# tachitachi/SR-WaveNet

Measured on NVIDIA B200. Metric: audio samples/sec, higher is better.
Workload: dtype f16

## Files before the change

sr-wavenet_b200/csrc/fused.cu:

```cuda
#include "common.cuh"
#include "mol.cuh"
#include "umma.cuh"
#include "philox.cuh"
#include <cuda_fp16.h>
#include <algorithm>
#include <cstdlib>

namespace fused {

constexpr int kTile = 128;
__host__ __device__ constexpr int tiles_of(bool teacher) { return teacher ? 3 : 4; }
__host__ __device__ constexpr int chunk_of(bool teacher) { return kTile * tiles_of(teacher); }
constexpr int kHalo = 512;
constexpr int kMaxLayers = 40;
constexpr int kMaxSeg = 8;

constexpr int kWfBytes = 64 * 32 * 2;
constexpr int kWrsTeacher = 32 * 160 * 2;
constexpr int kWrsStudent = 32 * 32 * 2;
constexpr int kH1Bytes = 128 * 128 * 2;
constexpr int kH2Bytes = 128 * 32 * 2;

struct Seg { int b, t_start, t_out, t_end; };

// ... 18 lines not shown
  int* err;
#ifdef SRWN_TUNING
  long long* trace;
  int trace_chunk;
#endif
  int T, L, P, frames, O, M;
  int ring_bytes_per_team;
  int dil[kMaxLayers];
  int ring_off[kMaxLayers];
  int rsuf[kMaxLayers + 1];
};

template <bool TEACHER>
struct SmemMapT {
  static constexpr int NT = tiles_of(TEACHER);
  static constexpr int rows = kHalo + NT * kTile;
  static constexpr int hbuf = 0;
  static constexpr int hbuf_bytes = 4 * rows * 16;
  static constexpr int cbuf = hbuf + 2 * hbuf_bytes;
  static constexpr int cbuf_bytes = 4 * kTile * 16;
  static constexpr int wst = cbuf + NT * cbuf_bytes;
  static constexpr int wst_bytes = kWfBytes + (TEACHER ? kWrsTeacher : kWrsStudent);
  static constexpr int head = wst + 2 * wst_bytes;
  static constexpr int bias = head + (TEACHER ? kH1Bytes + kH2Bytes : 0);
  static constexpr int hbias = bias + kMaxLayers * 32 * 4;
  static constexpr int front = hbias + (128 + 128 + 32 + 64 + 4) * 4;
  static constexpr int cbs = front + 64 * 4;
  static constexpr int bars = cbs + NT * (kMaxLayers + 1) * 32 * 4;
  static constexpr int n_bars = 40;
  static constexpr int misc = bars + n_bars * 8;
  static constexpr int total = misc + 64;
};
static_assert(SmemMapT<true>::total <= 232448 && SmemMapT<false>::total <= 232448, "shared memory budget");
static_assert(3 * 16 * kTile * 16 <= 2 * SmemMapT<true>::hbuf_bytes, "head operand overlay");

template <int NT>
struct BarT {
  static constexpr int D1 = 0;
  static constexpr int D2 = NT;
  static constexpr int HD = 2 * NT;
  static constexpr int WFULL = 4 * NT;
  static constexpr int WEMPTY = WFULL + 2;
  static constexpr int HALO = WFULL + 4;
  static constexpr int G1 = WFULL + 6;
  static constexpr int HDD = WFULL + 8;
  static constexpr int TAIL = HDD + NT;
  static constexpr int C2 = TAIL + 1;
  static constexpr int count = C2 + 2 * NT;
};
static_assert(BarT<3>::count <= 40 && BarT<4>::count <= 40, "barrier slots");

using namespace umma;

__device__ __forceinline__ uint32_t gate2(f2_t a) {
  float a0, a1;
  upk(a, a0, a1);
  const f2_t f = pk(tanh_fast(a0), tanh_fast(a1));
  const f2_t s = mul2(f, f);
  f2_t t = fma2(s, pk(0.0017294071149080992f, 0.0017294071149080992f), pk(-0.020638039335608482f, -0.020638039335608482f));
  t = fma2(s, t, pk(0.2499687224626541f, 0.2499687224626541f));
  const f2_t c = fma2(f, pk(0.5f, 0.5f), mul2(s, t));
  float c0, c1;
  upk(c, c0, c1);
  return pack2(c0, c1);
}

__device__ __forceinline__ void store_row(uint8_t* buf, int rows_per_kc, int row, const float* v) {
#pragma unroll
  for (int kc = 0; kc < 4; kc++) {
    uint4 q;
    q.x = pack2(v[kc * 8 + 0], v[kc * 8 + 1]); q.y = pack2(v[kc * 8 + 2], v[kc * 8 + 3]);
    q.z = pack2(v[kc * 8 + 4], v[kc * 8 + 5]); q.w = pack2(v[kc * 8 + 6], v[kc * 8 + 7]);
    *reinterpret_cast<uint4*>(buf + ((size_t)kc * rows_per_kc + row) * 16) = q;
  }
}
__device__ __forceinline__ void store_row_packed(uint8_t* buf, int rows_per_kc, int row, const uint32_t* w) {
#pragma unroll
  for (int kc = 0; kc < 4; kc++)
    *reinterpret_cast<uint4*>(buf + ((size_t)kc * rows_per_kc + row) * 16) =
        make_uint4(w[kc * 4 + 0], w[kc * 4 + 1], w[kc * 4 + 2], w[kc * 4 + 3]);
}

#ifndef SRWN_TUNING
#define TRACE(role, layer, slot) do {} while (0)
#else
#define TRACE(role, layer, slot)                                                            \
  do {                                                                                      \
    if (tracing) p.trace[((role) * kMaxLayers + (layer)) * 12 + (slot)] = clock64();      \
  } while (0)
#endif

constexpr int kLoadWarp = 0;
__host__ __device__ constexpr int threads_of(bool handoff, int nt) { return (1 + 4 * nt + (handoff ? 1 : 0)) * 32; }

__device__ __noinline__ bool flag_spin(const uint32_t* f, uint32_t need, volatile int* abort_flag, const int* gerr, int code, long long limit) {
  const long long t0 = clock64();
  int spins = 0;
  uint32_t v;
  while (true) {
    __nanosleep(32);
    asm volatile("ld.acquire.gpu.global.u32 %0, [%1];" : "=r"(v) : "l"(f) : "memory");
    if (v >= need) return true;
    if (*abort_flag) return false;
    if (((++spins) & 1023) == 0 && *reinterpret_cast<const volatile int*>(gerr)) return false;
    if (clock64() - t0 > limit) {
      if (atomicCAS((int*)abort_flag, 0, 1) == 0) ((int*)abort_flag)[1] = code;
      return false;
    }
  }
}
__device__ __forceinline__ bool flag_try(const uint32_t* f, uint32_t need) {
  uint32_t v;
  asm volatile("ld.acquire.gpu.global.u32 %0, [%1];" : "=r"(v) : "l"(f) : "memory");
  if (v < need) return false;
  asm volatile("fence.proxy.async;" ::: "memory");
  return true;
}
__device__ __forceinline__ bool flag_wait(const uint32_t* f, uint32_t need, volatile int* abort_flag, const int* gerr, int code, long long limit) {
  uint32_t v;
  asm volatile("ld.acquire.gpu.global.u32 %0, [%1];" : "=r"(v) : "l"(f) : "memory");
  if (v < need && !flag_spin(f, need, abort_flag, gerr, code, limit)) return false;
// ... 84 lines not shown

  const int G = p.G, team = (int)blockIdx.x / G, member = (int)blockIdx.x % G;
  const Seg* segs = p.segs + (size_t)team * kMaxSeg;
  const int nseg = p.nseg[team];
  uint8_t* ring = p.rings + (size_t)team * p.ring_bytes_per_team;
  uint32_t* flags = p.flags + (size_t)team * kMaxLayers;
  const uint32_t ringcnt = sbase + SM::misc + 16;
  uint32_t pub_expect = 0;
  int seq = 0;
  int u0e = 0, u0o = 0, lay_base = 0;
  int chunk_idx = 0;
  int head_idx = 0;
  int tail_idx = 0;
  double nll_acc = 0.0;
  const bool elected = elect_one();

  for (int si = 0; si < nseg; si++) {
    const Seg sg = segs[si];
    for (int t0 = sg.t_start; t0 < sg.t_end; t0 += CH) {
      const int n = seq++;
      if (n % G != member) continue;
      const bool warm = TEACHER ? (t0 + CH <= sg.t_out) : false;
      const bool do_head = TEACHER && !warm;
      int Lc = L;
      if (t0 + CH <= sg.t_out) {
        const int dist = sg.t_out - (t0 + CH);
        Lc = 0;
        while (Lc < L && p.rsuf[Lc + 1] > dist) Lc++;
        if (Lc < 1) Lc = 1;
      }
#define U0(par) ((par) ? u0o : u0e)
#ifdef SRWN_TUNING
      const bool tracing_chunk = p.trace != nullptr && blockIdx.x == 0 && chunk_idx == p.trace_chunk;
#else
      constexpr bool tracing_chunk = false; (void)tracing_chunk;
#endif

      if (warp == kLoadWarp) {
        bool have_next = false;
        for (int l = 0; l < Lc; l++) {
          const int s = l & 1;
          const int use = U0(s) + (l >> 1);
          [[maybe_unused]] const bool tracing = tracing_chunk && lane == 0;
          TRACE(6, l, 0);
          if (l >= 2 && !mbar_wait(bar(BAR_G1 + s), (use - 1) & 1, abort_flag, 0x1100000 | l, p.wait_limit)) break;
          TRACE(6, l, 2);
          if (HANDOFF && n > 0 && !have_next &&
              !flag_wait(flags + l, (uint32_t)n, abort_flag, p.err, 0x1200000 | l, p.wait_limit)) break;
          have_next = false;
          const int d = p.dil[l];
          const uint8_t* rl = ring + p.ring_off[l];
          const uint32_t dst0 = sbase + SM::hbuf + s * SM::hbuf_bytes;
          const int slot0 = (int)((unsigned)t0 % (unsigned)d);
          if (t0 - d >= sg.t_start) {
            if (lane == 0) {
              mbar_expect_tx(bar(BAR_HALO + s), (uint32_t)(4 * d * 16));
              const uint32_t n1 = (uint32_t)(d - slot0) * 16, n2 = (uint32_t)slot0 * 16;
#pragma unroll
              for (int kc = 0; kc < 4; kc++) {
                const uint32_t dst = dst0 + (uint32_t)(kc * ROWS + kHalo - d) * 16;
                const uint8_t* src = rl + (size_t)kc * d * 16;
                asm volatile("cp.async.bulk.shared::cluster.global.mbarrier::complete_tx::bytes [%0], [%1], %2, [%3];"
                             ::"r"(dst), "l"(src + (size_t)slot0 * 16), "r"(n1), "r"(bar(BAR_HALO + s)) : "memory");
                if (n2)
                  asm volatile("cp.async.bulk.shared::cluster.global.mbarrier::complete_tx::bytes [%0], [%1], %2, [%3];"
                               ::"r"(dst + n1), "l"(src), "r"(n2), "r"(bar(BAR_HALO + s)) : "memory");
// ... 40 lines not shown
            const int rows = ring_rows_of(p.dil[r], lane, CH);
            if (rows) {
              pub_expect += (uint32_t)rows;
              if ((int32_t)(ld_acquire_cta_shared(ringcnt + 4 * lane) - pub_expect) < 0) {
                const long long t0 = clock64();
                while ((int32_t)(ld_acquire_cta_shared(ringcnt + 4 * lane) - pub_expect) < 0) {
                  __nanosleep(128);
                  if (*abort_flag) { ok = false; break; }
                  if (clock64() - t0 > p.wait_limit) {
                    if (atomicCAS((int*)abort_flag, 0, 1) == 0) ((int*)abort_flag)[1] = 0x4000000 | (lane << 8) | r;
                    ok = false; break;
                  }
                }
              }
            }
          }
          ok = __all_sync(0xffffffffu, ok);
          if (ok && lane == 0) flag_publish(flags + r, (uint32_t)n + 1);
        }
        if (ok && lane == 0)
          for (int r = last + 1; r < L; r++) flag_publish(flags + r, (uint32_t)n + 1);
      } else {
        const int gw = warp & 3, m = (((warp - 1) >> 2) + gw + 1) % NT;
        const bool issuer = gw == m;
        const bool leader = issuer && elected;
        const int row = gw * 32 + lane;
        const uint32_t lane_addr = (uint32_t)(gw * 32) << 16;
        const int t = t0 + m * kTile + row;
        const bool in_utt = t < p.T;
        int frame = (t0 + m * kTile) / p.P;
        if (frame > p.frames - 1) frame = p.frames - 1;
        const float* cb_g = p.cb + ((size_t)sg.b * p.frames + frame) * (size_t)(L + 1) * 32;
        float* cb = reinterpret_cast<float*>(smem + SM::cbs) + m * (kMaxLayers + 1) * 32;
        for (int i = row; i < (L + 1) * 32; i += kTile) cb[i] = __ldg(cb_g + i);
        group_sync(m);
        const float* s_bias = reinterpret_cast<const float*>(smem + SM::bias);
        const float* s_front = reinterpret_cast<const float*>(smem + SM::front);
        const int rc = m * kTile + row;
        f2_t h2[16];
        float v[32];
        uint32_t w16[16];
        bool alive = true;
        [[maybe_unused]] const bool tracing = tracing_chunk && row == 0;
        constexpr uint32_t id32 = make_idesc(0, 128, 32), id128 = make_idesc(0, 128, 128);
        const uint32_t hb_lo0 = ((sbase + SM::hbuf) >> 4) + (uint32_t)(kHalo + m * kTile) + ((uint32_t)ROWS << 16);
        const uint32_t wb_lo0 = (sbase + SM::wst) >> 4;
        const uint32_t d_conv = tmem + m * TCOLS, d_skip = tmem + m * TCOLS + 32;
        uint32_t d_cop = d_skip;
        constexpr bool kLateG1 = !TEACHER && !HANDOFF;
        constexpr bool kLateWempty = !TEACHER && HANDOFF;

        {
          auto x_at = [&](int tt) -> float {
            const size_t i = (size_t)sg.b * p.T + tt;
            if (!TEACHER && p.noise.on) return philox::logistic_at(p.noise.seed, p.noise.stream, (uint64_t)i);
            return __ldg(p.x_in + i);
          };
          const float xm1 = (t >= 1 && t - 1 < p.T) ? x_at(t - 1) : 0.f;
          const float xm2 = (t >= 2 && t - 2 < p.T) ? x_at(t - 2) : 0.f;
#pragma unroll
          for (int j = 0; j < 16; j++) {
            const float a = fmaf(xm2, s_front[2 * j], fmaf(xm1, s_front[32 + 2 * j], cb[2 * j]));
            const float b = fmaf(xm2, s_front[2 * j + 1], fmaf(xm1, s_front[32 + 2 * j + 1], cb[2 * j + 1]));
            h2[j] = pk(a, b);
            w16[j] = pack2(a, b);
          }
          alive = mbar_wait(bar(BAR_HALO + 0), U0(0) & 1, abort_flag, 0x2000000 | (m << 8), p.wait_limit);
          store_row_packed(smem + SM::hbuf, ROWS, kHalo + rc, w16);
          const int d0 = p.dil[0];
          fence_async_smem();
          mbar_arrive(bar(BAR_HD + 2 * m + 0));
          if (rc >= CH - d0) store_row_packed(ring + p.ring_off[0], d0, t % d0, w16);
        }

        for (int l = 0; l < Lc; l++) {
          const int s = l & 1, sn = s ^ 1;
          const uint32_t ph = (lay_base + l) & 1, phs = (U0(s) + (l >> 1)) & 1;
          TRACE(m, l, 0);
          const uint32_t hb_lo = hb_lo0 + (uint32_t)(s * (SM::hbuf_bytes >> 4));
          const uint32_t wb_lo = wb_lo0 + (uint32_t)(s * (SM::wst_bytes >> 4));
          const uint32_t dl = (uint32_t)p.dil[l];
          const uint32_t b1_lo = wb_lo + (32u << 16);
          const uint32_t b2_lo = wb_lo + (kWfBytes >> 4) + ((uint32_t)wrs_rows << 16);
          if (gw == ((m + 3) & 3)) {
            alive = mbar_wait(bar(BAR_WFULL + s), phs, abort_flag, 0x3000000 | (m << 8) | l, p.wait_limit) && alive;
            if (NT > 3 && m >= 3) alive = mbar_wait(bar(BAR_HD + 2 * (m - 3) + s), phs, abort_flag, 0x3300000 | (m << 8) | l, p.wait_limit) && alive;
          }
          if (gw == ((m + 1) & 3) && m >= 1) alive = mbar_wait(bar(BAR_HD + 2 * (m - 1) + s), phs, abort_flag, 0x3100000 | (m << 8) | l, p.wait_limit) && alive;
          if (gw == ((m + 2) & 3) && m >= 2) alive = mbar_wait(bar(BAR_HD + 2 * (m - 2) + s), phs, abort_flag, 0x3200000 | (m << 8) | l, p.wait_limit) && alive;
          group_sync(m);
          TRACE(m, l, 1);
          if (HANDOFF && gw == (m == 0 ? 1 : 0) && lane == 0) {
            const int rows = ring_rows_of((int)dl, m, CH);
            if (rows) ring_rows_done(ringcnt + 4 * m, (uint32_t)rows);
          }
          if (issuer) {
            tc_fence_after();
            if (leader) {
              tc_mma<0>(d_conv, desc_from_lo(hb_lo - dl), desc_from_lo(b1_lo), id32);
              tc_mma<1>(d_conv, desc_from_lo(hb_lo - dl + 2 * ROWS), desc_from_lo(b1_lo + 64), id32);
              tc_mma<1>(d_conv, desc_from_lo(hb_lo), desc_from_lo(b1_lo + 128), id32);
              tc_mma<1>(d_conv, desc_from_lo(hb_lo + 2 * ROWS), desc_from_lo(b1_lo + 192), id32);
              tc_commit(bar(BAR_D1 + m));
              if constexpr (!kLateG1) tc_commit(bar(BAR_G1 + s));
            }
            __syncwarp();
          }
          TRACE(m, l, 2);
          bool next_ok = true;
          if (l + 1 < Lc && !issuer) {
            if (l >= 1) next_ok = mbar_poll(bar(BAR_G1 + sn), (U0(sn) + ((l - 1) >> 1)) & 1);
// ... 65 lines not shown
          TRACE(m, l, 9);
          if (l + 1 < L) {
#pragma unroll
            for (int j = 0; j < 16; j++) { float a, b; upk(h2[j], a, b); w16[j] = pack2(a, b); }
            if (l + 1 < Lc) {
              if (!next_ok) {
                if (l >= 1) alive = mbar_wait(bar(BAR_G1 + sn), (U0(sn) + ((l - 1) >> 1)) & 1, abort_flag, 0x2300000 | (m << 8) | l, p.wait_limit) && alive;
                alive = mbar_wait(bar(BAR_HALO + sn), (U0(sn) + ((l + 1) >> 1)) & 1, abort_flag, 0x2400000 | (m << 8) | l, p.wait_limit) && alive;
              }
              TRACE(m, l, 10);
              store_row_packed(smem + SM::hbuf + sn * SM::hbuf_bytes, ROWS, kHalo + rc, w16);
              tc_fence_before();
              fence_async_smem();
              mbar_arrive(bar(BAR_HD + 2 * m + sn));
            } else {
              tc_fence_before();
              alive = mbar_wait(bar(BAR_TAIL), tail_idx & 1, abort_flag, 0x2700000 | (m << 8) | l, p.wait_limit) && alive;
            }
            const int dn = p.dil[l + 1];
            if (rc >= CH - dn) store_row_packed(ring + p.ring_off[l + 1], dn, t % dn, w16);
            TRACE(m, l, 11);
          } else {
            tc_fence_before();
          }
        }

        if (TEACHER) {
          if (do_head) {
            const float* s_hb = reinterpret_cast<const float*>(smem + SM::hbias);
            uint8_t* a3 = smem + SM::hbuf + m * (16 * kTile * 16);
            const uint32_t a3_lo = ((sbase + SM::hbuf + m * (16 * kTile * 16)) >> 4) + ((uint32_t)kTile << 16);
            alive = mbar_wait(bar(BAR_G1 + ((L - 1) & 1)), (U0((L - 1) & 1) + ((L - 1) >> 1)) & 1, abort_flag, 0x2500000 | (m << 8), p.wait_limit) && alive;
            alive = mbar_wait(bar(BAR_WEMPTY + ((L - 1) & 1)), (U0((L - 1) & 1) + ((L - 1) >> 1)) & 1, abort_flag, 0x2510000 | (m << 8), p.wait_limit) && alive;
            tc_fence_after();
#pragma unroll 1
            for (int hs = 0; hs < 2; hs++) {
              for (int q = 0; q < 4; q++) {
                tc_ld32(d_skip + lane_addr + q * 32, v);
                tc_wait_ld();
#pragma unroll
                for (int j = 0; j < 32; j++) v[j] = fmaxf(v[j] + s_hb[hs * 128 + q * 32 + j], 0.f);
                store_row(a3 + (size_t)q * 4 * kTile * 16, kTile, row, v);
              }
              tc_fence_before();
              fence_async_smem();
              group_sync(m);
              if (issuer) {
                tc_fence_after();
                if (leader && !*abort_flag) {
                  const uint32_t wlo = ((sbase + SM::head + (hs == 0 ? 0 : kH1Bytes)) >> 4) + ((uint32_t)(hs == 0 ? 128 : 32) << 16);
                  const int nrows = hs == 0 ? 128 : 32;
#pragma unroll
                  for (int j = 0; j < 8; j++)
                    tc_mma_dyn(hs == 0 ? d_skip : d_conv, desc_from_lo(a3_lo + 2 * j * kTile), desc_from_lo(wlo + 2 * j * nrows),
                               hs == 0 ? id128 : id32, j);
                  tc_commit(bar(BAR_HDD + m));
                }
                __syncwarp();
              }
              alive = mbar_wait(bar(BAR_HDD + m), (head_idx * 2 + hs) & 1, abort_flag, 0x2600000 | (m << 8) | hs, p.wait_limit) && alive;
              tc_fence_after();
            }
            tc_ld32(d_conv + lane_addr, v);
            tc_wait_ld();
            tc_fence_before();
            if (alive && in_utt && t >= sg.t_out) {
#pragma unroll
              for (int j = 0; j < 32; j++) v[j] += s_hb[256 + j];
              const size_t at = (size_t)sg.b * p.T + t;
              float nl = 0.f;
              if (p.x_scored) {
                const float xs = __ldg(p.x_scored + at);
                if (p.M == 5) nl = mol_nll_fixed<5>(xs, v);
                else {
                  float lg[32];
#pragma unroll
                  for (int j = 0; j < 32; j++) lg[j] = v[j];
                  nl = mol_nll_one(xs, lg, p.M);
                }
              }
              if (p.logits_out) {
                float* dst = p.logits_out + at * p.O;
                if (p.O == 20) {
#pragma unroll
                  for (int j = 0; j < 5; j++)
                    reinterpret_cast<float4*>(dst)[j] = make_float4(v[4 * j], v[4 * j + 1], v[4 * j + 2], v[4 * j + 3]);
                } else {
#pragma unroll
                  for (int j = 0; j < 32; j++) if (j < p.O) dst[j] = v[j];
                }
              }
              if (p.x_scored) {
                if (p.nll_out) p.nll_out[at] = nl;
                nll_acc += (double)nl;
              }
            }
          }
        } else {
          const float* s_hb = reinterpret_cast<const float*>(smem + SM::hbias);
          const float* hk = s_hb + 288;
          float p0 = 0.f, p1 = 0.f;
#pragma unroll
          for (int j = 0; j < 16; j++) {
            float a, b;
            upk(h2[j], a, b);
            const float e0 = fmaxf(a, 0.f), e1 = fmaxf(b, 0.f);
            p0 = fmaf(e0, hk[4 * j], p0); p1 = fmaf(e0, hk[4 * j + 1], p1);
            p0 = fmaf(e1, hk[4 * j + 2], p0); p1 = fmaf(e1, hk[4 * j + 3], p1);
          }
          if (alive && in_utt && t >= sg.t_out) {
            const size_t at = (size_t)sg.b * p.T + t;
            const float sc = expf(p0 + hk[64]);
            const float mu = p1 + hk[65];
            p.scale_out[at] = sc;
            p.mean_out[at] = mu;
            const float xin = p.noise.on ? philox::logistic_at(p.noise.seed, p.noise.stream, (uint64_t)at) : __ldg(p.x_in + at);
            p.x_out[at] = fmaf(xin, sc, mu);
          }
        }
      }
      if (HANDOFF && Lc < L && warp != kLoadWarp && warp != kPubWarp) {
        const int gw = warp & 3, m = (((warp - 1) >> 2) + gw + 1) % NT;
        group_sync(m);
        if (gw == (m == 0 ? 1 : 0) && lane == 0) {
          const int rows = ring_rows_of(p.dil[Lc], m, CH);
          if (rows) ring_rows_done(ringcnt + 4 * m, (uint32_t)rows);
        }
      }
      if (do_head) head_idx++;
      if (Lc < L) tail_idx++;
      chunk_idx++;
      u0e += (Lc + 1) >> 1; u0o += Lc >> 1; lay_base += Lc;
      tc_fence_before();
      asm volatile("fence.proxy.async;" ::: "memory");
      __syncthreads();
      tc_fence_after();
      if (*abort_flag) break;
    }
    if (*abort_flag) break;
  }

  if (TEACHER && p.nll_partial) {
    double* s_red = reinterpret_cast<double*>(smem + SM::cbuf);
    for (int s = 16; s >= 1; s >>= 1) nll_acc += __shfl_xor_sync(0xffffffffu, nll_acc, s);
    if (lane == 0) s_red[warp] = nll_acc;
    __syncthreads();
    if (tid == 0) {
      double tot = 0;
      for (int w = 1; w <= 4 * NT; w++) tot += s_red[w];
      p.nll_partial[blockIdx.x] = tot;
    }
  }
  if (tid == 0 && *abort_flag) {
    volatile int* e = p.err;
    e[1] = abort_flag[1]; e[2] = chunk_idx; e[3] = blockIdx.x;
    __threadfence_system();
    e[0] = 1;
  }
  tc_fence_before();
  __syncthreads();
  if (warp == kLoadWarp) {
    tc_fence_after();
    asm volatile("tcgen05.dealloc.cta_group::1.sync.aligned.b32 %0, %1;" ::"r"(tmem), "r"(512));
  }
}

__global__ void k_sum_partials(const double* __restrict__ part, int n, float* __restrict__ out) {
  double tot = 0;
  for (int i = threadIdx.x; i < n; i += 32) tot += part[i];
// ... 236 lines not shown
    if (force_G > 0 && G != std::min(force_G, std::min(kMaxTeam, grid))) continue;
    int teams = grid / G;
    if ((long long)teams > total) teams = (int)total;
    if (teams < 1) continue;
    Partition cand = partition_for(B, T, kChunk, warm_cost, teams);
    const double lag = kLagLayers / L;
    const double period = std::max(1.0, G * lag);
    const double time = (cand.cost / G + (G > 1 ? 0.5 : 0.0)) * period * (G > 1 ? handoff_cost : 1.0) + (G - 1) * lag;
    if (time < best_time) { best_time = time; best = cand; best.G = G; }
  }
  return best;
}

struct FusedWs {
  float* cb; uint8_t* rings; uint32_t* flags; double* partial;
#ifdef SRWN_TUNING
  long long* trace;
#endif
  float *scales, *means, *xa, *xb;
  size_t bytes;
};

static FusedWs carve_fused(const srwn_ctx* c, int B, int T, void* ws, size_t cap) {
  WsCarver w(ws, cap);
  FusedWs r{};
  const size_t frames = T / c->cfg.pool_stride, L = c->cfg.n_layers, n = (size_t)B * T;
  const int grid = c->sm_count > 0 ? c->sm_count : 148;
  const size_t nst = c->cfg.kind == SRWN_STUDENT ? (size_t)c->cfg.num_flows : 1;
  r.cb = w.take<float>((size_t)B * frames * (L + 1) * 32 * nst);
  r.rings = w.take<uint8_t>((size_t)grid * ((size_t)c->sum_dilation * 64 + 256));
  r.flags = w.take<uint32_t>((size_t)grid * kMaxLayers * nst);
  r.partial = w.take<double>(grid);
#ifdef SRWN_TUNING
  r.trace = w.take<long long>(7 * kMaxLayers * 12);
#endif
  if (c->cfg.kind == SRWN_STUDENT) {
    r.scales = w.take<float>(n * c->cfg.num_flows);
    r.means = w.take<float>(n * c->cfg.num_flows);
    r.xa = w.take<float>(n);
    r.xb = w.take<float>(n);
  }
  r.bytes = w.used;
  return r;
}

size_t fused_partition_bytes(const srwn_ctx* c) {
  const size_t grid = c->sm_count > 0 ? c->sm_count : 148;
  return grid * kMaxSeg * sizeof(Seg) + grid * sizeof(int);
}

size_t fused_workspace_bytes(const srwn_ctx* c, int op, int B, int T) {
  return carve_fused(c, B, T, nullptr, 0).bytes;
}

template <bool TEACHER>
static int launch_fused(srwn_ctx* c, const Params& p, int grid, cudaStream_t st) {
  const bool handoff = p.G > 1;
  auto kern = handoff ? k_fused<TEACHER, true> : k_fused<TEACHER, false>;
  SRWN_CUDA(cudaFuncSetAttribute(kern, cudaFuncAttributeMaxDynamicSharedMemorySize, SmemMapT<TEACHER>::total));
  Params pl = p;
  void* args[] = {&pl};
  SRWN_CUDA(cudaLaunchCooperativeKernel((const void*)kern, dim3(grid), dim3(threads_of(handoff, tiles_of(TEACHER))), args, SmemMapT<TEACHER>::total, st));
  SRWN_LAUNCH_CHECK();
  return SRWN_OK;
}

static int sticky_error(const srwn_ctx* c) {
// ... 90 lines not shown
  for (int f = 0; f < F; f++) {
    Params p;
    int rc = prepare(c, f, enc, B, T, w, &p, &grid, f == 0, st);
    if (rc) return rc;
    float* xout = (f == F - 1 && x_last) ? x_last : ((f & 1) ? w.xb : w.xa);
    p.x_in = xin; p.scale_out = w.scales + (size_t)f * n; p.mean_out = w.means + (size_t)f * n; p.x_out = xout;
    if (f == 0) p.noise = noise;
    ProfScope prof(c, st, "k_fused<student,fp16>", 1);
    rc = launch_fused<false>(c, p, grid, st);
    if (rc) return rc;
    xin = xout;
  }
  return run_flow_compose(z, noise, z_out, w.scales, w.means, F, out, s_tot, mu_tot, (int64_t)n, st);
}

int fused_check_error(void* ws, size_t ws_bytes, const srwn_ctx* c, int B, int T, cudaStream_t st) {
  (void)ws; (void)ws_bytes; (void)B; (void)T;
  SRWN_CUDA(cudaStreamSynchronize(st));
  volatile int* e = c->h_err;
  if (e && e[0]) {
    const int code = e[1], chunk = e[2], cta = e[3];
    e[0] = 0; e[1] = 0; e[2] = 0; e[3] = 0;
    return srwn_fail(SRWN_ERR_CUDA, "fused kernel aborted: pipeline wait timed out (code 0x%x, chunk %d, cta %d)", code, chunk, cta);
  }
  return SRWN_OK;
}

void fused_last_partition(const srwn_ctx* c, int* teams, int* G) { *teams = c->part_teams; *G = c->part_G; }

#ifdef SRWN_TUNING
extern "C" int srwn_debug_read_trace(srwn_handle_t h, int32_t B, int32_t T, void* ws, size_t ws_bytes,
                                     long long* out, int32_t count) {
  FusedWs w = carve_fused(h, B, T, ws, ws_bytes);
  if (count > 7 * kMaxLayers * 12) count = 7 * kMaxLayers * 12;
  SRWN_CUDA(cudaDeviceSynchronize());
  SRWN_CUDA(cudaMemcpy(out, w.trace, sizeof(long long) * count, cudaMemcpyDeviceToHost));
  return SRWN_OK;
}

namespace fused {
template <int N, int CNT>
__device__ __forceinline__ void bench_issue(uint32_t tmem_col, uint32_t a_lo, uint32_t b_lo, uint32_t mbar_addr) {
  constexpr uint32_t idesc = make_idesc(0, 128, N);
#pragma unroll
  for (int i = 0; i < CNT; i++) {
    if (i == 0) tc_mma<0>(tmem_col, desc_from_lo(a_lo), desc_from_lo(b_lo), idesc);
    else tc_mma<1>(tmem_col, desc_from_lo(a_lo + (i & 3) * 256), desc_from_lo(b_lo + (i & 3) * 64), idesc);
  }
  tc_commit(mbar_addr);
}

__global__ void __launch_bounds__(416, 1) k_mma_bench(long long* out) {
  extern __shared__ __align__(1024) uint8_t smem[];
  __shared__ uint32_t tmem_slot;
  __shared__ __align__(8) uint64_t mbar[16];
  __shared__ long long s_t[16][2];
  const uint32_t sbase = smem_u32(smem);
  const int warp = threadIdx.x >> 5;
  for (int i = threadIdx.x; i < 65536 / 4; i += 416) reinterpret_cast<uint32_t*>(smem)[i] = 0x3c003c00u;
  if (threadIdx.x == 0) {
    for (int i = 0; i < 16; i++) mbar_init(smem_u32(&mbar[i]), 1);
    asm volatile("fence.mbarrier_init.release.cluster;" ::: "memory");
  }
  fence_async_smem();
  if (warp == 0) {
    asm volatile("tcgen05.alloc.cta_group::1.sync.aligned.shared::cta.b32 [%0], %1;" ::"r"(smem_u32(&tmem_slot)), "r"(512));
    asm volatile("tcgen05.relinquish_alloc_permit.cta_group::1.sync.aligned;" ::);
// ... 61 lines not shown
```

sr-wavenet_b200/csrc/mol.cu:

```cuda
#include "common.cuh"
#include "mol.cuh"

constexpr int kMaxRedBlocks = 2048;

__global__ void __launch_bounds__(256)
k_mol_loss(const float* __restrict__ x, const float* __restrict__ l, float* __restrict__ nll_out,
           double* __restrict__ partial, int64_t n, int M) {
  double local = 0.0;
  for (int64_t i = (int64_t)blockIdx.x * blockDim.x + threadIdx.x; i < n;
       i += (int64_t)gridDim.x * blockDim.x) {
    float lg[kMaxLogit];
    const float* li = l + i * 4 * M;
    for (int j = 0; j < 3 * M; j++) lg[j] = li[j];
    const float v = mol_nll_one(x[i], lg, M);
    if (nll_out) nll_out[i] = v;
    local += (double)v;
  }
  if (!partial) return;
  __shared__ double s_part[8];
  for (int s = 16; s >= 1; s >>= 1) local += __shfl_xor_sync(0xffffffffu, local, s);
  if ((threadIdx.x & 31) == 0) s_part[threadIdx.x >> 5] = local;
  __syncthreads();
  if (threadIdx.x == 0) {
    double b = 0;
    for (int w = 0; w < 8; w++) b += s_part[w];
    partial[blockIdx.x] = b;
  }
}

__global__ void k_mol_loss_sum(const double* __restrict__ partial, int n, float* __restrict__ nll_sum) {
  if (threadIdx.x == 0 && blockIdx.x == 0) {
    double tot = 0;
    for (int i = 0; i < n; i++) tot += partial[i];
    *nll_sum = (float)tot;
  }
}

int run_mol_loss(const float* x, const float* l, float* nll_out, float* nll_sum, int B, int T, int M,
                 cudaStream_t st) {
  if (M < 1 || 4 * M > kMaxLogit) return srwn_fail(SRWN_ERR_UNSUPPORTED, "num_mixtures must be 1..%d", kMaxLogit / 4);
  const int64_t n = (int64_t)B * T;
  int64_t blocks = (n + 255) / 256;
  if (blocks > kMaxRedBlocks) blocks = kMaxRedBlocks;
  double* partial = nullptr;
  if (nll_sum) SRWN_CUDA(cudaMallocAsync((void**)&partial, (size_t)blocks * sizeof(double), st));
  k_mol_loss<<<(unsigned)blocks, 256, 0, st>>>(x, l, nll_out, partial, n, M);
  SRWN_LAUNCH_CHECK();
// ... 31 lines not shown
```

sr-wavenet_b200/csrc/mol.cuh:

```cuda
#pragma once
#include <cuda_runtime.h>

__device__ __forceinline__ float srwn_softplus(float x) {
  return fmaxf(x, 0.f) + log1pf(expf(-fabsf(x)));
}

__device__ __forceinline__ float mol_nll_one(float x, const float* lg, int M) {
  float mx = lg[0];
  for (int m = 1; m < M; m++) mx = fmaxf(mx, lg[m]);
  float se = 0.f;
  for (int m = 0; m < M; m++) se += expf(lg[m] - mx);
  const float lse_p = mx + logf(se);
  float lp[8];
  float best = -INFINITY;
  for (int m = 0; m < M; m++) {
    const float mean = lg[M + m];
    const float ls = fmaxf(lg[2 * M + m], -7.f);
    const float inv = expf(-ls);
    const float c = x - mean;
    const float plus = inv * (c + 1.f / 255.f);
    const float mn = inv * (c - 1.f / 255.f);
    const float mid = inv * c;
    float v;
    if (x < -0.999f) {
      v = plus - srwn_softplus(plus);
    } else if (x > 0.999f) {
      v = -srwn_softplus(mn);
    } else {
      float a = plus, b = mn;
      if (mid > 0.f) { a = -mn; b = -plus; }
      const float ea = expf(a), eb = expf(b);
      const float delta = -ea * expm1f(b - a) / ((1.f + ea) * (1.f + eb));
      if (delta > 1e-5f) v = logf(fmaxf(delta, 1e-12f));
      else v = mid - ls - 2.f * srwn_softplus(mid) - 4.8481163902538321f;
    }
    v += lg[m] - lse_p;
    lp[m] = v;
    best = fmaxf(best, v);
  }
  float s = 0.f;
  for (int m = 0; m < M; m++) s += expf(lp[m] - best);
  return -(best + logf(s));
}

template <int M>
__device__ __forceinline__ float mol_nll_fixed(float x, const float* lg) {
  float mx = lg[0];
#pragma unroll
  for (int m = 1; m < M; m++) mx = fmaxf(mx, lg[m]);
  float se = 0.f;
#pragma unroll
  for (int m = 0; m < M; m++) se += expf(lg[m] - mx);
  const float lse_p = mx + logf(se);
  float lp[M];
  float best = -INFINITY;
#pragma unroll
  for (int m = 0; m < M; m++) {
    const float mean = lg[M + m];
    const float ls = fmaxf(lg[2 * M + m], -7.f);
    const float inv = expf(-ls);
    const float c = x - mean;
    const float plus = inv * (c + 1.f / 255.f);
    const float mn = inv * (c - 1.f / 255.f);
    const float mid = inv * c;
    float v;
    if (x < -0.999f) {
      v = plus - srwn_softplus(plus);
    } else if (x > 0.999f) {
      v = -srwn_softplus(mn);
    } else {
      float a = plus, b = mn;
      if (mid > 0.f) { a = -mn; b = -plus; }
      const float ea = expf(a), eb = expf(b);
      const float delta = -ea * expm1f(b - a) / ((1.f + ea) * (1.f + eb));
      if (delta > 1e-5f) v = logf(fmaxf(delta, 1e-12f));
      else v = mid - ls - 2.f * srwn_softplus(mid) - 4.8481163902538321f;
    }
    v += lg[m] - lse_p;
    lp[m] = v;
    best = fmaxf(best, v);
  }
  float s = 0.f;
#pragma unroll
  for (int m = 0; m < M; m++) s += expf(lp[m] - best);
  return -(best + logf(s));
}

__device__ __forceinline__ float mol_sample_one(const float* lg, const float* u1, float u2, int M,
                                                int* k_out) {
  int k = 0;
  float best = -INFINITY;
  for (int m = 0; m < M; m++) {
    const float v = lg[m] - logf(-logf(u1[m]));
    if (v > best) { best = v; k = m; }
  }
  const float mean = lg[M + k];
  const float ls = fmaxf(lg[2 * M + k], -7.f);
  float x = mean + expf(ls) * (logf(u2) - logf(1.f - u2));
  x = fminf(fmaxf(x, -1.f), 1.f);
  *k_out = k;
  return x;
}
```

sr-wavenet_b200/csrc/umma.cuh:

```cuda
#pragma once
#include <cuda_fp16.h>
#include <stdint.h>

namespace umma {

__device__ __forceinline__ uint32_t smem_u32(const void* p) { return (uint32_t)__cvta_generic_to_shared(p); }

__device__ __forceinline__ void mbar_init(uint32_t a, uint32_t count) {
  asm volatile("mbarrier.init.shared::cta.b64 [%0], %1;" ::"r"(a), "r"(count));
}
__device__ __forceinline__ void mbar_arrive(uint32_t a) {
  asm volatile("mbarrier.arrive.shared::cta.b64 _, [%0];" ::"r"(a) : "memory");
}
__device__ __forceinline__ void mbar_expect_tx(uint32_t a, uint32_t bytes) {
  asm volatile("mbarrier.arrive.expect_tx.shared::cta.b64 _, [%0], %1;" ::"r"(a), "r"(bytes) : "memory");
}
__device__ __forceinline__ bool mbar_test(uint32_t a, uint32_t parity) {
  uint32_t ok;
  asm volatile("{\n\t.reg .pred p;\n\tmbarrier.try_wait.parity.shared::cta.b64 p, [%1], %2;\n\t"
               "selp.u32 %0, 1, 0, p;\n\t}" : "=r"(ok) : "r"(a), "r"(parity) : "memory");
  return ok != 0;
}
__device__ __forceinline__ bool mbar_poll(uint32_t a, uint32_t parity) {
  uint32_t ok;
// ... 52 lines not shown
__device__ __forceinline__ void tc_mma_ts(uint32_t d_tmem, uint32_t a_tmem, uint64_t b, uint32_t idesc) {
  asm volatile("{\n\t.reg .pred p;\n\tsetp.ne.b32 p, %4, 0;\n\t"
               "tcgen05.mma.cta_group::1.kind::f16 [%0], [%1], %2, %3, p;\n\t}"
               ::"r"(d_tmem), "r"(a_tmem), "l"(b), "r"(idesc), "n"(ACC) : "memory");
}
__device__ __forceinline__ void tc_mma_ts_dyn(uint32_t d_tmem, uint32_t a_tmem, uint64_t b, uint32_t idesc, uint32_t acc) {
  asm volatile("{\n\t.reg .pred p;\n\tsetp.ne.b32 p, %4, 0;\n\t"
               "tcgen05.mma.cta_group::1.kind::f16 [%0], [%1], %2, %3, p;\n\t}"
               ::"r"(d_tmem), "r"(a_tmem), "l"(b), "r"(idesc), "r"(acc) : "memory");
}
__device__ __forceinline__ void tc_st16(uint32_t taddr, const uint32_t* r) {
  asm volatile("tcgen05.st.sync.aligned.32x32b.x16.b32 [%0], "
               "{%1, %2, %3, %4, %5, %6, %7, %8, %9, %10, %11, %12, %13, %14, %15, %16};"
               ::"r"(taddr), "r"(r[0]), "r"(r[1]), "r"(r[2]), "r"(r[3]), "r"(r[4]), "r"(r[5]), "r"(r[6]), "r"(r[7]),
                 "r"(r[8]), "r"(r[9]), "r"(r[10]), "r"(r[11]), "r"(r[12]), "r"(r[13]), "r"(r[14]), "r"(r[15]) : "memory");
}
__device__ __forceinline__ void tc_wait_st() { asm volatile("tcgen05.wait::st.sync.aligned;" ::: "memory"); }
__device__ __forceinline__ void tc_wait_ld() { asm volatile("tcgen05.wait::ld.sync.aligned;" ::: "memory"); }

__device__ __forceinline__ uint64_t desc_from_lo(uint32_t lo) { return ((uint64_t)0x4008u << 32) | lo; }
__device__ __forceinline__ uint64_t make_desc(uint32_t saddr, uint32_t lbo_bytes, uint32_t sbo_bytes) {
  return (uint64_t)((saddr >> 4) & 0x3FFF) | ((uint64_t)((lbo_bytes >> 4) & 0x3FFF) << 16) |
         ((uint64_t)((sbo_bytes >> 4) & 0x3FFF) << 32) | ((uint64_t)1 << 46);
}
__host__ __device__ constexpr uint32_t make_idesc(int fmt, int M, int N) {
  return (1u << 4) | ((uint32_t)fmt << 7) | ((uint32_t)fmt << 10) | ((uint32_t)(N >> 3) << 17) | ((uint32_t)(M >> 4) << 24);
}

__device__ __forceinline__ uint32_t pack2(float a, float b) {
  uint32_t r;
  asm("cvt.rn.satfinite.f16x2.f32 %0, %1, %2;" : "=r"(r) : "f"(b), "f"(a));
  return r;
}
__device__ __forceinline__ bool elect_one() {
  uint32_t pred;
  asm volatile("{\n\t.reg .pred P;\n\telect.sync _|P, 0xffffffff;\n\tselp.u32 %0, 1, 0, P;\n\t}" : "=r"(pred));
  return pred != 0;
}
__device__ __forceinline__ float tanh_fast(float x) {
  float y;
  asm("tanh.approx.f32 %0, %1;" : "=f"(y) : "f"(x));
  return y;
}

typedef unsigned long long f2_t;
__device__ __forceinline__ f2_t pk(float lo, float hi) { f2_t r; asm("mov.b64 %0, {%1, %2};" : "=l"(r) : "f"(lo), "f"(hi)); return r; }
__device__ __forceinline__ void upk(f2_t v, float& lo, float& hi) { asm("mov.b64 {%0, %1}, %2;" : "=f"(lo), "=f"(hi) : "l"(v)); }
__device__ __forceinline__ f2_t fma2(f2_t a, f2_t b, f2_t c) { f2_t r; asm("fma.rn.f32x2 %0, %1, %2, %3;" : "=l"(r) : "l"(a), "l"(b), "l"(c)); return r; }
__device__ __forceinline__ f2_t add2(f2_t a, f2_t b) { f2_t r; asm("add.rn.f32x2 %0, %1, %2;" : "=l"(r) : "l"(a), "l"(b)); return r; }
__device__ __forceinline__ f2_t mul2(f2_t a, f2_t b) { f2_t r; asm("mul.rn.f32x2 %0, %1, %2;" : "=l"(r) : "l"(a), "l"(b)); return r; }


}
```

Measured before the change: 913.1 million.

## Overlap head TMEM loads, async-copy conditioning, and approximate MoL loss math

Conditioning rows now come from global memory through cp.async, and the front input samples are loaded while those copies are in flight. The head's skip-path loop double-buffers tcgen05 loads, loading the next 32 columns while the current ones get bias, packed ReLU and the store. The ReLU is folded into the f16 conversion. The mixture-of-logistics NLL is rewritten with approximate ex2/lg2/rcp, a polynomial expm1 and branchless edge handling. Together these aim to hide load latency and cut special-function cost in the head, at the risk of small numeric differences in the loss. Tracing instrumentation is also added.

```diff
diff --git a/sr-wavenet_b200/csrc/fused.cu b/sr-wavenet_b200/csrc/fused.cu
--- a/sr-wavenet_b200/csrc/fused.cu
+++ b/sr-wavenet_b200/csrc/fused.cu
@@ -74,6 +74,7 @@
   static constexpr int total = misc + 64;
 };
 static_assert(SmemMapT<true>::total <= 232448 && SmemMapT<false>::total <= 232448, "shared memory budget");
+static_assert(SmemMapT<true>::cbs % 16 == 0 && SmemMapT<false>::cbs % 16 == 0, "conditioning rows are copied in 16-byte pieces");
 static_assert(3 * 16 * kTile * 16 <= 2 * SmemMapT<true>::hbuf_bytes, "head operand overlay");
 
 template <int NT>
@@ -107,15 +108,6 @@
   return pack2(c0, c1);
 }
 
-__device__ __forceinline__ void store_row(uint8_t* buf, int rows_per_kc, int row, const float* v) {
-#pragma unroll
-  for (int kc = 0; kc < 4; kc++) {
-    uint4 q;
-    q.x = pack2(v[kc * 8 + 0], v[kc * 8 + 1]); q.y = pack2(v[kc * 8 + 2], v[kc * 8 + 3]);
-    q.z = pack2(v[kc * 8 + 4], v[kc * 8 + 5]); q.w = pack2(v[kc * 8 + 6], v[kc * 8 + 7]);
-    *reinterpret_cast<uint4*>(buf + ((size_t)kc * rows_per_kc + row) * 16) = q;
-  }
-}
 __device__ __forceinline__ void store_row_packed(uint8_t* buf, int rows_per_kc, int row, const uint32_t* w) {
 #pragma unroll
   for (int kc = 0; kc < 4; kc++)
@@ -125,10 +117,21 @@
 
 #ifndef SRWN_TUNING
 #define TRACE(role, layer, slot) do {} while (0)
+#define TRACE_HEAD(tile, slot) do {} while (0)
+#define TRACE_NEXT(tile, slot) do {} while (0)
 #else
+constexpr int kTraceWords = (7 * kMaxLayers + 4) * 12;
 #define TRACE(role, layer, slot)                                                            \
   do {                                                                                      \
     if (tracing) p.trace[((role) * kMaxLayers + (layer)) * 12 + (slot)] = clock64();      \
+  } while (0)
+#define TRACE_HEAD(tile, slot)                                                              \
+  do {                                                                                      \
+    if (tracing) p.trace[(7 * kMaxLayers + (tile)) * 12 + (slot)] = clock64();            \
+  } while (0)
+#define TRACE_NEXT(tile, slot)                                                              \
+  do {                                                                                      \
+    if (tracing_next) p.trace[(7 * kMaxLayers + (tile)) * 12 + (slot)] = clock64();       \
   } while (0)
 #endif
 
@@ -279,6 +282,7 @@
 #define U0(par) ((par) ? u0o : u0e)
 #ifdef SRWN_TUNING
       const bool tracing_chunk = p.trace != nullptr && blockIdx.x == 0 && chunk_idx == p.trace_chunk;
+      const bool tracing_next_chunk = p.trace != nullptr && blockIdx.x == 0 && chunk_idx == p.trace_chunk + 1;
 #else
       constexpr bool tracing_chunk = false; (void)tracing_chunk;
 #endif
@@ -385,7 +389,16 @@
         if (frame > p.frames - 1) frame = p.frames - 1;
         const float* cb_g = p.cb + ((size_t)sg.b * p.frames + frame) * (size_t)(L + 1) * 32;
         float* cb = reinterpret_cast<float*>(smem + SM::cbs) + m * (kMaxLayers + 1) * 32;
-        for (int i = row; i < (L + 1) * 32; i += kTile) cb[i] = __ldg(cb_g + i);
+        for (int i = row; i < (L + 1) * 8; i += kTile)
+          asm volatile("cp.async.cg.shared.global [%0], [%1], 16;" ::"r"(smem_u32(cb + 4 * i)), "l"(cb_g + 4 * i) : "memory");
+        auto x_at = [&](int tt) -> float {
+          const size_t i = (size_t)sg.b * p.T + tt;
+          if (!TEACHER && p.noise.on) return philox::logistic_at(p.noise.seed, p.noise.stream, (uint64_t)i);
+          return __ldg(p.x_in + i);
+        };
+        const float xm1 = (t >= 1 && t - 1 < p.T) ? x_at(t - 1) : 0.f;
+        const float xm2 = (t >= 2 && t - 2 < p.T) ? x_at(t - 2) : 0.f;
+        asm volatile("cp.async.wait_all;" ::: "memory");
         group_sync(m);
         const float* s_bias = reinterpret_cast<const float*>(smem + SM::bias);
         const float* s_front = reinterpret_cast<const float*>(smem + SM::front);
@@ -395,6 +408,9 @@
         uint32_t w16[16];
         bool alive = true;
         [[maybe_unused]] const bool tracing = tracing_chunk && row == 0;
+#ifdef SRWN_TUNING
+        const bool tracing_next = tracing_next_chunk && row == 0;
+#endif
         constexpr uint32_t id32 = make_idesc(0, 128, 32), id128 = make_idesc(0, 128, 128);
         const uint32_t hb_lo0 = ((sbase + SM::hbuf) >> 4) + (uint32_t)(kHalo + m * kTile) + ((uint32_t)ROWS << 16);
         const uint32_t wb_lo0 = (sbase + SM::wst) >> 4;
@@ -404,13 +420,6 @@
         constexpr bool kLateWempty = !TEACHER && HANDOFF;
 
         {
-          auto x_at = [&](int tt) -> float {
-            const size_t i = (size_t)sg.b * p.T + tt;
-            if (!TEACHER && p.noise.on) return philox::logistic_at(p.noise.seed, p.noise.stream, (uint64_t)i);
-            return __ldg(p.x_in + i);
-          };
-          const float xm1 = (t >= 1 && t - 1 < p.T) ? x_at(t - 1) : 0.f;
-          const float xm2 = (t >= 2 && t - 2 < p.T) ? x_at(t - 2) : 0.f;
 #pragma unroll
           for (int j = 0; j < 16; j++) {
             const float a = fmaf(xm2, s_front[2 * j], fmaf(xm1, s_front[32 + 2 * j], cb[2 * j]));
@@ -420,6 +429,7 @@
           }
           alive = mbar_wait(bar(BAR_HALO + 0), U0(0) & 1, abort_flag, 0x2000000 | (m << 8), p.wait_limit);
           store_row_packed(smem + SM::hbuf, ROWS, kHalo + rc, w16);
+          if (TEACHER) TRACE_NEXT(m, 7);
           const int d0 = p.dil[0];
           fence_async_smem();
           mbar_arrive(bar(BAR_HD + 2 * m + 0));
@@ -430,6 +440,7 @@
           const int s = l & 1, sn = s ^ 1;
           const uint32_t ph = (lay_base + l) & 1, phs = (U0(s) + (l >> 1)) & 1;
           TRACE(m, l, 0);
+          if (TEACHER && l == 0) TRACE_NEXT(m, 8);
           const uint32_t hb_lo = hb_lo0 + (uint32_t)(s * (SM::hbuf_bytes >> 4));
           const uint32_t wb_lo = wb_lo0 + (uint32_t)(s * (SM::wst_bytes >> 4));
           const uint32_t dl = (uint32_t)p.dil[l];
@@ -561,19 +572,39 @@
             const uint32_t a3_lo = ((sbase + SM::hbuf + m * (16 * kTile * 16)) >> 4) + ((uint32_t)kTile << 16);
             alive = mbar_wait(bar(BAR_G1 + ((L - 1) & 1)), (U0((L - 1) & 1) + ((L - 1) >> 1)) & 1, abort_flag, 0x2500000 | (m << 8), p.wait_limit) && alive;
             alive = mbar_wait(bar(BAR_WEMPTY + ((L - 1) & 1)), (U0((L - 1) & 1) + ((L - 1) >> 1)) & 1, abort_flag, 0x2510000 | (m << 8), p.wait_limit) && alive;
+            TRACE_HEAD(m, 0);
             tc_fence_after();
 #pragma unroll 1
             for (int hs = 0; hs < 2; hs++) {
-              for (int q = 0; q < 4; q++) {
-                tc_ld32(d_skip + lane_addr + q * 32, v);
+              auto relu_pack_store = [&](const float* u, int q) {
+                const ulonglong2* hb2 = reinterpret_cast<const ulonglong2*>(s_hb + hs * 128 + q * 32);
+#pragma unroll
+                for (int k = 0; k < 8; k++) {
+                  const ulonglong2 bb = hb2[k];
+                  float e0, e1, e2, e3;
+                  upk(add2(pk(u[4 * k], u[4 * k + 1]), bb.x), e0, e1);
+                  upk(add2(pk(u[4 * k + 2], u[4 * k + 3]), bb.y), e2, e3);
+                  w16[2 * k] = pack2_relu(e0, e1);
+                  w16[2 * k + 1] = pack2_relu(e2, e3);
+                }
+                store_row_packed(a3 + (size_t)q * 4 * kTile * 16, kTile, row, w16);
+              };
+              float u[32];
+              tc_ld32(d_skip + lane_addr, v);
+              tc_wait_ld();
+#pragma unroll
+              for (int q = 0; q < 4; q += 2) {
+                tc_ld32(d_skip + lane_addr + (q + 1) * 32, u);
+                relu_pack_store(v, q);
                 tc_wait_ld();
-#pragma unroll
-                for (int j = 0; j < 32; j++) v[j] = fmaxf(v[j] + s_hb[hs * 128 + q * 32 + j], 0.f);
-                store_row(a3 + (size_t)q * 4 * kTile * 16, kTile, row, v);
+                if (q + 2 < 4) tc_ld32(d_skip + lane_addr + (q + 2) * 32, v);
+                relu_pack_store(u, q + 1);
+                if (q + 2 < 4) tc_wait_ld();
               }
               tc_fence_before();
               fence_async_smem();
               group_sync(m);
+              TRACE_HEAD(m, 1 + 2 * hs);
               if (issuer) {
                 tc_fence_after();
                 if (leader && !*abort_flag) {
@@ -588,6 +619,7 @@
                 __syncwarp();
               }
               alive = mbar_wait(bar(BAR_HDD + m), (head_idx * 2 + hs) & 1, abort_flag, 0x2600000 | (m << 8) | hs, p.wait_limit) && alive;
+              TRACE_HEAD(m, 2 + 2 * hs);
               tc_fence_after();
             }
             tc_ld32(d_conv + lane_addr, v);
@@ -600,12 +632,12 @@
               float nl = 0.f;
               if (p.x_scored) {
                 const float xs = __ldg(p.x_scored + at);
-                if (p.M == 5) nl = mol_nll_fixed<5>(xs, v);
+                if (p.M == 5) nl = mol_nll<5>(xs, v, 5);
                 else {
                   float lg[32];
 #pragma unroll
                   for (int j = 0; j < 32; j++) lg[j] = v[j];
-                  nl = mol_nll_one(xs, lg, p.M);
+                  nl = mol_nll<kMaxLogit / 4>(xs, lg, p.M);
                 }
               }
               if (p.logits_out) {
@@ -624,6 +656,7 @@
                 nll_acc += (double)nl;
               }
             }
+            TRACE_HEAD(m, 5);
           }
         } else {
           const float* s_hb = reinterpret_cast<const float*>(smem + SM::hbias);
@@ -664,6 +697,10 @@
       asm volatile("fence.proxy.async;" ::: "memory");
       __syncthreads();
       tc_fence_after();
+#ifdef SRWN_TUNING
+      if (TEACHER && tracing_chunk && warp != kLoadWarp && !(HANDOFF && warp == kPubWarp) && (warp & 3) == 0 && lane == 0)
+        p.trace[(7 * kMaxLayers + (((warp - 1) >> 2) + 1) % NT) * 12 + 6] = clock64();
+#endif
       if (*abort_flag) break;
     }
     if (*abort_flag) break;
@@ -966,7 +1003,7 @@
   r.flags = w.take<uint32_t>((size_t)grid * kMaxLayers * nst);
   r.partial = w.take<double>(grid);
 #ifdef SRWN_TUNING
-  r.trace = w.take<long long>(7 * kMaxLayers * 12);
+  r.trace = w.take<long long>(kTraceWords);
 #endif
   if (c->cfg.kind == SRWN_STUDENT) {
     r.scales = w.take<float>(n * c->cfg.num_flows);
@@ -1123,7 +1160,7 @@
 extern "C" int srwn_debug_read_trace(srwn_handle_t h, int32_t B, int32_t T, void* ws, size_t ws_bytes,
                                      long long* out, int32_t count) {
   FusedWs w = carve_fused(h, B, T, ws, ws_bytes);
-  if (count > 7 * kMaxLayers * 12) count = 7 * kMaxLayers * 12;
+  if (count > kTraceWords) count = kTraceWords;
   SRWN_CUDA(cudaDeviceSynchronize());
   SRWN_CUDA(cudaMemcpy(out, w.trace, sizeof(long long) * count, cudaMemcpyDeviceToHost));
   return SRWN_OK;
diff --git a/sr-wavenet_b200/csrc/mol.cu b/sr-wavenet_b200/csrc/mol.cu
--- a/sr-wavenet_b200/csrc/mol.cu
+++ b/sr-wavenet_b200/csrc/mol.cu
@@ -12,7 +12,7 @@
     float lg[kMaxLogit];
     const float* li = l + i * 4 * M;
     for (int j = 0; j < 3 * M; j++) lg[j] = li[j];
-    const float v = mol_nll_one(x[i], lg, M);
+    const float v = mol_nll<kMaxLogit / 4>(x[i], lg, M);
     if (nll_out) nll_out[i] = v;
     local += (double)v;
   }
diff --git a/sr-wavenet_b200/csrc/mol.cuh b/sr-wavenet_b200/csrc/mol.cuh
--- a/sr-wavenet_b200/csrc/mol.cuh
+++ b/sr-wavenet_b200/csrc/mol.cuh
@@ -5,85 +5,65 @@
   return fmaxf(x, 0.f) + log1pf(expf(-fabsf(x)));
 }
 
-__device__ __forceinline__ float mol_nll_one(float x, const float* lg, int M) {
-  float mx = lg[0];
-  for (int m = 1; m < M; m++) mx = fmaxf(mx, lg[m]);
+__device__ __forceinline__ float mol_ex2(float x) { float y; asm("ex2.approx.ftz.f32 %0, %1;" : "=f"(y) : "f"(x)); return y; }
+__device__ __forceinline__ float mol_lg2(float x) { float y; asm("lg2.approx.ftz.f32 %0, %1;" : "=f"(y) : "f"(x)); return y; }
+__device__ __forceinline__ float mol_rcp(float x) { float y; asm("rcp.approx.ftz.f32 %0, %1;" : "=f"(y) : "f"(x)); return y; }
+constexpr float kMolLog2e = 1.4426950408889634f, kMolLn2 = 0.69314718055994531f;
+
+__device__ __forceinline__ float mol_softplus(float y) {
+  return fmaxf(y, 0.f) + kMolLn2 * mol_lg2(1.f + mol_ex2(-fabsf(y) * kMolLog2e));
+}
+
+__device__ __forceinline__ float mol_expm1_neg(float z) {
+  float p = fmaf(z, 1.f / 720.f, 1.f / 120.f);
+  p = fmaf(z, p, 1.f / 24.f);
+  p = fmaf(z, p, 1.f / 6.f);
+  p = fmaf(z, p, 0.5f);
+  p = fmaf(z, p, 1.f);
+  const float e = mol_ex2(z * kMolLog2e) - 1.f;
+  return z > -0.25f ? z * p : e;
+}
+
+template <int MAXM>
+__device__ __forceinline__ float mol_nll(float x, const float* lg, int M) {
+  float mx = -INFINITY;
+#pragma unroll
+  for (int m = 0; m < MAXM; m++) if (m < M) mx = fmaxf(mx, lg[m]);
+  const float mxs = mx * kMolLog2e;
   float se = 0.f;
-  for (int m = 0; m < M; m++) se += expf(lg[m] - mx);
-  const float lse_p = mx + logf(se);
-  float lp[8];
+#pragma unroll
+  for (int m = 0; m < MAXM; m++) if (m < M) se += mol_ex2(fmaf(lg[m], kMolLog2e, -mxs));
+  const float lse_p = fmaf(mol_lg2(se), kMolLn2, mx);
+  const bool lo_edge = x < -0.999f, hi_edge = x > 0.999f;
+  float lp[MAXM];
   float best = -INFINITY;
-  for (int m = 0; m < M; m++) {
+#pragma unroll
+  for (int m = 0; m < MAXM; m++) {
+    if (m >= M) break;
     const float mean = lg[M + m];
     const float ls = fmaxf(lg[2 * M + m], -7.f);
-    const float inv = expf(-ls);
+    const float inv = mol_ex2(-ls * kMolLog2e);
     const float c = x - mean;
     const float plus = inv * (c + 1.f / 255.f);
     const float mn = inv * (c - 1.f / 255.f);
     const float mid = inv * c;
-    float v;
-    if (x < -0.999f) {
-      v = plus - srwn_softplus(plus);
-    } else if (x > 0.999f) {
-      v = -srwn_softplus(mn);
-    } else {
-      float a = plus, b = mn;
-      if (mid > 0.f) { a = -mn; b = -plus; }
-      const float ea = expf(a), eb = expf(b);
-      const float delta = -ea * expm1f(b - a) / ((1.f + ea) * (1.f + eb));
-      if (delta > 1e-5f) v = logf(fmaxf(delta, 1e-12f));
-      else v = mid - ls - 2.f * srwn_softplus(mid) - 4.8481163902538321f;
-    }
-    v += lg[m] - lse_p;
+    const bool flip = mid > 0.f;
+    const float a = flip ? -mn : plus, b = flip ? -plus : mn;
+    const float ea = mol_ex2(a * kMolLog2e), eb = mol_ex2(b * kMolLog2e);
+    const float delta = -ea * mol_expm1_neg(mn - plus) * mol_rcp((1.f + ea) * (1.f + eb));
+    const float sp = mol_softplus(lo_edge ? plus : (hi_edge ? mn : mid));
+    const float v_in = delta > 1e-5f ? kMolLn2 * mol_lg2(delta)
+                                     : mid - ls - 2.f * sp - 4.8481163902538321f;
+    const float v_edge = (lo_edge ? plus : 0.f) - sp;
+    const float v = ((lo_edge || hi_edge) ? v_edge : v_in) + (lg[m] - lse_p);
     lp[m] = v;
     best = fmaxf(best, v);
   }
-  float s = 0.f;
-  for (int m = 0; m < M; m++) s += expf(lp[m] - best);
-  return -(best + logf(s));
-}
-
-template <int M>
-__device__ __forceinline__ float mol_nll_fixed(float x, const float* lg) {
-  float mx = lg[0];
-#pragma unroll
-  for (int m = 1; m < M; m++) mx = fmaxf(mx, lg[m]);
-  float se = 0.f;
-#pragma unroll
-  for (int m = 0; m < M; m++) se += expf(lg[m] - mx);
-  const float lse_p = mx + logf(se);
-  float lp[M];
-  float best = -INFINITY;
-#pragma unroll
-  for (int m = 0; m < M; m++) {
-    const float mean = lg[M + m];
-    const float ls = fmaxf(lg[2 * M + m], -7.f);
-    const float inv = expf(-ls);
-    const float c = x - mean;
-    const float plus = inv * (c + 1.f / 255.f);
-    const float mn = inv * (c - 1.f / 255.f);
-    const float mid = inv * c;
-    float v;
-    if (x < -0.999f) {
-      v = plus - srwn_softplus(plus);
-    } else if (x > 0.999f) {
-      v = -srwn_softplus(mn);
-    } else {
-      float a = plus, b = mn;
-      if (mid > 0.f) { a = -mn; b = -plus; }
-      const float ea = expf(a), eb = expf(b);
-      const float delta = -ea * expm1f(b - a) / ((1.f + ea) * (1.f + eb));
-      if (delta > 1e-5f) v = logf(fmaxf(delta, 1e-12f));
-      else v = mid - ls - 2.f * srwn_softplus(mid) - 4.8481163902538321f;
-    }
-    v += lg[m] - lse_p;
-    lp[m] = v;
-    best = fmaxf(best, v);
-  }
+  const float bs = best * kMolLog2e;
   float s = 0.f;
 #pragma unroll
-  for (int m = 0; m < M; m++) s += expf(lp[m] - best);
-  return -(best + logf(s));
+  for (int m = 0; m < MAXM; m++) if (m < M) s += mol_ex2(fmaf(lp[m], kMolLog2e, -bs));
+  return -fmaf(mol_lg2(s), kMolLn2, best);
 }
 
 __device__ __forceinline__ float mol_sample_one(const float* lg, const float* u1, float u2, int M,
diff --git a/sr-wavenet_b200/csrc/umma.cuh b/sr-wavenet_b200/csrc/umma.cuh
--- a/sr-wavenet_b200/csrc/umma.cuh
+++ b/sr-wavenet_b200/csrc/umma.cuh
@@ -108,6 +108,11 @@
   asm("cvt.rn.satfinite.f16x2.f32 %0, %1, %2;" : "=r"(r) : "f"(b), "f"(a));
   return r;
 }
+__device__ __forceinline__ uint32_t pack2_relu(float a, float b) {
+  uint32_t r;
+  asm("cvt.rn.satfinite.relu.f16x2.f32 %0, %1, %2;" : "=r"(r) : "f"(b), "f"(a));
+  return r;
+}
 __device__ __forceinline__ bool elect_one() {
   uint32_t pred;
   asm volatile("{\n\t.reg .pred P;\n\telect.sync _|P, 0xffffffff;\n\tselp.u32 %0, 1, 0, P;\n\t}" : "=r"(pred));
```

Result: no change. 920.7 million (median of 6 runs) (+0.8%).
